# CANGA/ELMKernels

Hardware: AMD Instinct MI355X
Metric: gridcell-timesteps/sec (higher is better)
Workload: dtype f64

## Files before the change

### elmkernels_amd/csrc/elmk_albedo_col.h

```cpp
#pragma once
#include "elmk_dev.h"

namespace elmk {

#ifndef LV
#define LV(f, lev) S->f[(int64_t)(lev) * ld + c]
#endif

constexpr double SN_MIN_SNW = 1.0e-30;
constexpr double SA_MPE = 1.e-06;
constexpr double SA_EXTKN = 0.30;

__device__ __forceinline__ int alb_main_column(const DevState* __restrict__ S, const int64_t c, const int64_t ld, const Land& L)
{
  const double coszen = S->coszen[c];
  const double elai = S->elai[c];

  S->nrad[c] = 1;
  S->tlai_z[c] = elai;

  if (!(coszen > 0.0)) return -1;

  const double h2osno = S->h2osno[c];
  const int snl = S->snl[c];

  double albsod[2], albsoi[2];
  {
    const double albice[2] = {0.8, 0.55};
    const double alblak[2] = {0.60, 0.40};
    const double alblakwi[2] = {0.10, 0.10};
    if (L.ltype == istsoil || L.ltype == istcrop) {
      const int col = S->isoicol[c];
      const double inc = dmax(0.11 - 0.40 * LV(h2osoi_vol, 0), 0.0);
#pragma unroll
      for (int ib = 0; ib < 2; ib++) {
        albsod[ib] = dmin(S->albsat[col][ib] + inc, S->albdry[col][ib]);
        albsoi[ib] = albsod[ib];
      }
    } else if (L.ltype == istice || L.ltype == istice_mec) {
#pragma unroll
      for (int ib = 0; ib < 2; ib++) {
        albsod[ib] = albice[ib];
        albsoi[ib] = albsod[ib];
      }
    } else if (L.ltype == istdlak && snl == 0) {
      const double t_grnd = S->t_grnd[c];
      const double sicefr = 1.0 - elmk_exp(-95.6 * (TFRZ - t_grnd) / TFRZ);
#pragma unroll
      for (int ib = 0; ib < 2; ib++) {
        albsod[ib] = sicefr * alblak[ib] + (1.0 - sicefr) * dmax(alblakwi[ib], 0.05 / (dmax(0.001, coszen) + 0.15));
        albsoi[ib] = sicefr * alblak[ib] + (1.0 - sicefr) * dmax(alblakwi[ib], 0.10);
      }
    } else {
#pragma unroll
      for (int ib = 0; ib < 2; ib++) {
        albsod[ib] = alblak[ib];
        albsoi[ib] = albsod[ib];
      }
    }
  }


  LV(albsod, 0) = albsod[0];
  LV(albsod, 1) = albsod[1];
  LV(albsoi, 0) = albsoi[0];
  LV(albsoi, 1) = albsoi[1];
  if (h2osno > SN_MIN_SNW) return snl == 0 ? 1 : snl;
  return 0;
}

}
```

### elmkernels_amd/csrc/elmk_albedo_fin.h

```cpp
#pragma once
#include "elmk_dev.h"
#include "elmk_albedo_col.h"

namespace elmk {

struct AlbFwd {
  double albsod[2], albsoi[2], albsnd[2], albsni[2], albgrd[2], albgri[2];
  double albd[2], albi[2], ftdd[2], ftid[2], ftii[2], fabd[2], fabi[2];
  double fsun_z, fabd_sun_z, fabd_sha_z, fabi_sun_z, fabi_sha_z;
};

__device__ __forceinline__ void alb_ground(const DevState* __restrict__ S, const int64_t c, const int64_t ld, const bool day,
                                           const double frac_sno, const double (&albsod)[2], const double (&albsoi)[2],
                                           const double (&sd_alb)[2], const double (&si_alb)[2], AlbFwd& a)
{
#pragma unroll
  for (int ib = 0; ib < 2; ib++) {
    double o_sod = 0.0, o_soi = 0.0, o_snd = 0.0, o_sni = 0.0, g_d = 0.0, g_i = 0.0;
    if (day) {
      g_d = albsod[ib] * (1.0 - frac_sno) + sd_alb[ib] * frac_sno;
      g_i = albsoi[ib] * (1.0 - frac_sno) + si_alb[ib] * frac_sno;
      o_sod = albsod[ib];
      o_soi = albsoi[ib];
      o_snd = sd_alb[ib];
// ... 172 lines not shown
        fabi_sha_z = fabi_sha[ib] / ((1.0 - fsun_z) * laisum);
        const double extkb = twostext;
        vcmaxcintsun = (1.0 - elmk_exp(-(SA_EXTKN + extkb) * elai)) / (SA_EXTKN + extkb);
        vcmaxcintsha = (1.0 - elmk_exp(-SA_EXTKN * elai)) / SA_EXTKN - vcmaxcintsun;
        if (elai > 0.0) {
          vcmaxcintsun = vcmaxcintsun / (fsun_z * elai);
          vcmaxcintsha = vcmaxcintsha / ((1.0 - fsun_z) * elai);
        } else {
          vcmaxcintsun = 0.0;
          vcmaxcintsha = 0.0;
        }
      }
    }
  } else {
#pragma unroll
    for (int ib = 0; ib < 2; ++ib) {
      fabd[ib] = 0.0;
      fabi[ib] = 0.0;
      fabi_sun[ib] = 0.0;
      fabi_sha[ib] = 0.0;
      ftdd[ib] = 1.0;
      ftid[ib] = 0.0;
      ftii[ib] = 1.0;
      albd[ib] = albgrd[ib];
      albi[ib] = albgri[ib];
    }
  }
#pragma unroll
  for (int ib = 0; ib < 2; ib++) {
    LV(albd, ib) = albd[ib];
    LV(albi, ib) = albi[ib];
    LV(ftdd, ib) = ftdd[ib];
    LV(ftid, ib) = ftid[ib];
    LV(ftii, ib) = ftii[ib];
    LV(fabd, ib) = fabd[ib];
    LV(fabi, ib) = fabi[ib];
    LV(fabi_sun, ib) = fabi_sun[ib];
    LV(fabi_sha, ib) = fabi_sha[ib];
  }
  S->vcmaxcintsun[c] = vcmaxcintsun;
  S->vcmaxcintsha[c] = vcmaxcintsha;
  S->fsun_z[c] = fsun_z;
  S->fabd_sun_z[c] = fabd_sun_z;
  S->fabd_sha_z[c] = fabd_sha_z;
  S->fabi_sun_z[c] = fabi_sun_z;
  S->fabi_sha_z[c] = fabi_sha_z;
}

struct AlbIn {
  bool day, snicar;
  double coszen, elai, esai, frac_sno, vcmaxcintsun, vcmaxcintsha;
  double albsod[2], albsoi[2], sd_alb[2], si_alb[2];
};
__device__ __forceinline__ AlbIn alb_final_inputs(const DevState* __restrict__ S, const int64_t c, const int64_t ld, const double frac_sno_in,
                                                  const double h2osno_in)
{
  AlbIn x;
  x.coszen = S->coszen[c];
  x.elai = S->elai[c];
  x.vcmaxcintsun = 0.0;
  x.vcmaxcintsha = (1.0 - elmk_exp(-SA_EXTKN * x.elai)) / SA_EXTKN;
  if (x.elai > 0.0) {
    x.vcmaxcintsha /= x.elai;
  } else {
    x.vcmaxcintsha = 0.0;
  }
  x.day = x.coszen > 0.0;
  x.snicar = false;
  x.esai = 0.0;
  x.frac_sno = 0.0;
  x.albsod[0] = x.albsod[1] = x.albsoi[0] = x.albsoi[1] = 0.0;
  x.sd_alb[0] = x.sd_alb[1] = x.si_alb[0] = x.si_alb[1] = 0.0;
  if (x.day) {
    x.esai = S->esai[c];
    x.frac_sno = frac_sno_in;
    x.albsod[0] = LV(albsod, 0);
    x.albsod[1] = LV(albsod, 1);
    x.albsoi[0] = LV(albsoi, 0);
    x.albsoi[1] = LV(albsoi, 1);
    if (h2osno_in > SN_MIN_SNW) {
      const gptr<const double> o = S->alb_snow + c;
      x.snicar = true;
      x.sd_alb[0] = __builtin_nontemporal_load(o);
      x.sd_alb[1] = __builtin_nontemporal_load(o + ld);
      x.si_alb[0] = __builtin_nontemporal_load(o + (int64_t)14 * ld);
      x.si_alb[1] = __builtin_nontemporal_load(o + (int64_t)15 * ld);
    } else if (h2osno_in < SN_MIN_SNW && h2osno_in > 0.0) {
      x.sd_alb[0] = x.si_alb[0] = x.albsoi[0];
      x.sd_alb[1] = x.si_alb[1] = x.albsoi[1];
    }
  }
  return x;
}
__device__ __forceinline__ void alb_flux_abs_all(const DevState* __restrict__ S, const int64_t c, const int64_t ld, const Land& L,
                                                 const AlbIn& x, double (&flx)[6][4])
{
  const gptr<const double> o = S->alb_snow + c;
#pragma unroll
  for (int i = 0; i < 6; i++) {
    double sdf[2] = {0.0, 0.0}, sif[2] = {0.0, 0.0};
    if (x.snicar) {
      sdf[0] = __builtin_nontemporal_load(o + (int64_t)(2 + 2 * i) * ld);
      sdf[1] = __builtin_nontemporal_load(o + (int64_t)(3 + 2 * i) * ld);
      sif[0] = __builtin_nontemporal_load(o + (int64_t)(16 + 2 * i) * ld);
      sif[1] = __builtin_nontemporal_load(o + (int64_t)(17 + 2 * i) * ld);
    }
    alb_flux_abs_level(L, x.day, x.frac_sno, x.albsod, x.albsoi, x.sd_alb, x.si_alb, sdf, sif, flx[i][0], flx[i][1], flx[i][2], flx[i][3]);
    LV(flx_absdv, i) = flx[i][0];
    LV(flx_absdn, i) = flx[i][1];
    LV(flx_absiv, i) = flx[i][2];
    LV(flx_absin, i) = flx[i][3];
  }
}

}
```

### elmkernels_amd/csrc/elmk_api.cpp

```cpp
#include "elmk.h"

#include <hip/hip_runtime.h>

#include <cmath>
#include <cstddef>
#include <cstdio>
#include <cstdlib>
#include <algorithm>
#include <cstring>
#include <dlfcn.h>
#include <string>
#include <vector>

#include "elmk_dev.h"
#include "elmk_kernels.h"
#include "elmk_maps.h"

using namespace elmk;

namespace {

struct FieldDesc {
  const char* name;
  int dtype;
// ... 476 lines not shown
  }
  if (side.fork) (void)hipEventDestroy(side.fork);
  for (hipEvent_t e : done)
    if (e) (void)hipEventDestroy(e);
  if (upload) (void)hipStreamDestroy(upload);
  if (own) (void)hipStreamDestroy(own);
  return ELMK_OK;
}

const char* elmk_last_error(const elmk_ctx* ctx) { return ctx ? ctx->err.c_str() : g_create_error.c_str(); }

int elmk_set_stream(elmk_ctx* ctx, void* hip_stream)
{
  if (int rc = enter(ctx)) return rc;
  HIPCHK(hipStreamSynchronize(ctx->stream));
  ctx->stream = hip_stream ? (hipStream_t)hip_stream : ctx->own_stream;
  return ELMK_OK;
}

namespace {
int drop_graphs(elmk_ctx* ctx)
{
  HIPCHK(hipStreamSynchronize(ctx->stream));
  for (GraphSlot& g : ctx->graph) g.drop();
  return ELMK_OK;
}

int set_col_dayl(elmk_ctx* ctx, bool on)
{
  if (ctx->side.col_dayl == on) return ELMK_OK;
  if (int rc = drop_graphs(ctx)) return rc;
  ctx->side.col_dayl = on;
  return ELMK_OK;
}

int refuse_capture(elmk_ctx* ctx, const char* msg)
{
  hipStreamCaptureStatus cap = hipStreamCaptureStatusNone;
  if (hip_fail(ctx, hipStreamIsCapturing(ctx->stream, &cap), "hipStreamIsCapturing")) return ELMK_E_HIP;
  return cap != hipStreamCaptureStatusNone ? invalid(ctx, msg) : ELMK_OK;
}
}

int elmk_set_graph(elmk_ctx* ctx, int on)
{
  if (int rc = enter(ctx)) return rc;
  ctx->use_graph = on != 0;
  return ctx->use_graph ? ELMK_OK : drop_graphs(ctx);
}

int elmk_set_option(elmk_ctx* ctx, int option, int value)
{
  if (int rc = enter(ctx)) return rc;
  if (option != ELMK_OPT_CF_HALF_WORKGROUPS) return invalid(ctx, "elmk_set_option: unknown option");
  int cus = 0;
  HIPCHK(hipDeviceGetAttribute(&cus, hipDeviceAttributeMultiprocessorCount, ctx->dev));
  const int want = value ? (cus > 0 ? cus : 256) : 0;
  if (want != ctx->side.cf_half_groups) {
    if (int rc = drop_graphs(ctx)) return rc;
    ctx->side.cf_half_groups = want;
  }
  return ELMK_OK;
}

int elmk_sync(elmk_ctx* ctx)
{
  if (int rc = enter(ctx)) return rc;
  HIPCHK(hipStreamSynchronize(ctx->stream));
  return ELMK_OK;
}

int64_t elmk_ncols(const elmk_ctx* ctx) { return ctx ? ctx->ncols : -1; }
int64_t elmk_level_stride(const elmk_ctx* ctx) { return ctx ? ctx->ld : -1; }
int64_t elmk_device_bytes(const elmk_ctx* ctx)
{
  if (!ctx) return -1;
  size_t n = ctx->arena.bytes() + ctx->staging.bytes() + ctx->scratch.bytes() + ctx->snicar.bytes() + ctx->snowage.bytes() + ctx->d.bytes() +
             ctx->run.mem.bytes() + ctx->grid.mem.bytes() + ctx->ogrid.mem.bytes() + ctx->sw.czf.bytes() + ctx->run.rec.bytes() +
             ctx->ds.topo.bytes() + ctx->ds.gmem.bytes() + ctx->accum_table.bytes() + ctx->aer.mem.bytes();
  for (const elmk_ctx::HistEntry& e : ctx->hist) n += e.cells ? e.acc.bytes() : 0;
  for (const elmk_ctx::AccumEntry& e : ctx->accum) n += e.val.bytes();
  return (int64_t)n;
}

int elmk_num_fields(void) { return ELMK_NUM_FIELDS; }
const char* elmk_field_name(int field) { return field_ok(field) ? g_fields[field].name : nullptr; }
int elmk_field_id(const char* name)
{
  if (!name) return -1;
  for (int f = 0; f < ELMK_NUM_FIELDS; f++)
    if (strcmp(name, g_fields[f].name) == 0) return f;
  return -1;
}
int elmk_field_info(int field, int* nlev, int* dtype)
{
  if (!field_ok(field)) return ELMK_E_INVALID;
  if (nlev) *nlev = g_fields[field].nlev;
  if (dtype) *dtype = g_fields[field].dtype;
  return ELMK_OK;
}

static int xfer_rows(elmk_ctx* ctx, char* dev, int64_t ld, int es, int nlev, void* host, int64_t col0, int64_t n, int layout, bool up)
{
  if (layout == ELMK_LAYOUT_SOA || nlev == 1) {
    if (up)
      HIPCHK(hipMemcpy2DAsync(dev + (size_t)col0 * es, (size_t)ld * es, host, (size_t)n * es, (size_t)n * es, nlev, hipMemcpyHostToDevice,
// ... 2207 lines not shown
```

### elmkernels_amd/csrc/elmk_kernels.h

```cpp
#pragma once

#include <hip/hip_runtime.h>
#include <stdint.h>

#include "elmk.h"
#include "elmk_solar.h"

namespace elmk {

struct DevState;

constexpr int ELMK_NSIDE = 5;
struct SideStreams {
  hipStream_t s[ELMK_NSIDE];
  hipEvent_t fork;
  hipEvent_t join[ELMK_NSIDE];
  int cf_half_groups;
  bool one_stream;
  bool col_dayl;
};

void launch_frac_wet(const DevState* S, int64_t n, hipStream_t st);
void launch_albedo_snicar(const DevState* S, int64_t n, hipStream_t st, const SideStreams* side, bool fused = false);
unsigned launch_albedo_snicar_part(const DevState* S, int64_t n, hipStream_t st);
void launch_canopy_hydrology(const DevState* S, int64_t n, double dt, hipStream_t st);
void launch_surface_radiation(const DevState* S, int64_t n, hipStream_t st);
void launch_canopy_temperature(const DevState* S, int64_t n, hipStream_t st);
constexpr int GIVEN_FUSED = 1 << 8;
void launch_bareground_fluxes(const DevState* S, int64_t n, hipStream_t st, int given = 0);
void launch_canopy_fluxes(const DevState* S, int64_t n, double dt, hipStream_t st, int given = 0, const SideStreams* side = nullptr);
constexpr int ELMK_FUSED_NSTAGE = 5;
void launch_fused_stage(const DevState* S, int64_t n, double dt, hipStream_t st, const SideStreams* side, int stage);
void launch_bareground_list(const DevState* S, int64_t n, hipStream_t st);
void launch_soil_temperature(const DevState* S, int64_t n, double dt, hipStream_t st);
void launch_snow_hydrology(const DevState* S, int64_t n, double dt, hipStream_t st);
constexpr int ELMK_CONS_NPART = 512;
void launch_surface_fluxes(const DevState* S, int64_t n, double dt, hipStream_t st);
void launch_init_timestep(const DevState* S, int64_t n, hipStream_t st);
void launch_initialize_state(const DevState* S, int64_t n, hipStream_t st);
struct DsParams {
  const double* hc;
  const double* hf;
  double* lg;
  double lapse, lapse_lw, lw_limit;
};
void launch_get_forcing(const DevState* S, int64_t n, const double* wt1, const double* wt2, int qbot_is_rh, hipStream_t st,
                        const double* czf = nullptr, const DsParams* ds = nullptr);
void launch_phenology(const DevState* S, int64_t n, double wt1, double wt2, hipStream_t st);
void launch_conservation(const DevState* S, int64_t n, int64_t ld, double dt, const double* diag, double* part, double* out,
                         hipStream_t st);

void launch_cols_to_soa(const void* staging, void* field, int elem, int nlev, int64_t ld, int64_t col0, int64_t n,
                        hipStream_t st);
void launch_soa_to_cols(const void* field, void* staging, int elem, int nlev, int64_t ld, int64_t col0, int64_t n,
                        hipStream_t st);
constexpr int ELMK_F32_STORED = 16;
void launch_fill(void* field, int dtype, int nlev, int64_t ld, int64_t ncols, double value, hipStream_t st);
void launch_tile(void* field, int dtype, int nlev, int64_t ld, int64_t ncols, int64_t nbase, uint64_t seed,
                 int field_id, int mode, double amp, hipStream_t st);
void launch_flag_reduce(const uint32_t* flags, int64_t n, uint32_t* or_out, long long* first_bad, hipStream_t st);
void launch_copy(const double* src, double* dst, int64_t n, hipStream_t st, int shape = 0);
constexpr int COPY_JOBS_MAX = 16;
struct CopyJobs {
  const double* src[COPY_JOBS_MAX];
  double* dst[COPY_JOBS_MAX];
  int64_t end[COPY_JOBS_MAX];
  int n;
};
void launch_copy_multi(const CopyJobs& J, hipStream_t st);
void launch_math_eval(int fn, const double* x, const double* y, double* out, int64_t n, hipStream_t st);
// ... 107 lines not shown
```

### elmkernels_amd/csrc/elmk_snicar.h

```cpp
#pragma once
#include "elmk_dev.h"
#include "elmk_albedo_col.h"

namespace elmk {

constexpr int SN_RDS_MAX_TBL = 1500, SN_RDS_MIN_TBL = 30;
constexpr double SN_EXP_MIN = 4.5399929762484854e-05;

struct SnowOut {
  double alb[2];
  double fabs_[6][2];
};

template <int NL>
__device__ __forceinline__ void snicar_band(const DevState* __restrict__ S, const int64_t c, const int64_t ld, const int pass,
                                            const int bnd, const double mu_not, const int snl, const double h2osno,
                                            const double albsoi_b, double& albedo, double (&fl)[6], uint32_t& err)
{
  constexpr int snl_top = 5 - NL;
  const gptr<const double> tab = S->snicar;
  const double difgauspt[8] = {0.9894009, 0.9445750, 0.8656312, 0.7554044, 0.6178762, 0.4580168, 0.2816036, 0.0950125};
  const double difgauswt[8] = {0.0271525, 0.0622535, 0.0951585, 0.1246290, 0.1495960, 0.1691565, 0.1826034, 0.1894506};
  const double puny = 1.0e-11;
  const double c0 = 0.0, c1 = 1.0, c3 = 3.0, c4 = 4.0, cp5 = 0.5, cp75 = 0.75, c1p5 = 1.5, trmin = 0.001;
// ... 226 lines not shown

template <int NL, class FA, class FF>
__device__ __forceinline__ void snicar_combine_from(const int pass, const double mu_not, const int rds_top, const FA band_albedo,
                                                    const FF band_flux, SnowOut& out)
{
  constexpr int snl_top = 5 - NL;
  const double w1 = (pass == 0) ? 0.49352158521175 : 0.58581507618433;
  const double w2 = (pass == 0) ? 0.18099494230665 : 0.20156903770812;
  const double w3 = (pass == 0) ? 0.12094898498813 : 0.10917889346386;
  const double w4 = (pass == 0) ? 0.20453448749347 : 0.10343699264369;
  const double flx_wgt[5] = {1.0, w1, w2, w3, w4};
  double alb_nir_sum = 0.0, wgt_sum = 0.0;
  double nir_sum[6] = {0.0, 0.0, 0.0, 0.0, 0.0, 0.0};
  out.alb[0] = band_albedo(0);
#pragma unroll
  for (int i = 0; i < 6; i++) {
    out.fabs_[i][0] = band_flux(0, i);
    out.fabs_[i][1] = 0.0;
  }
#pragma unroll
  for (int b = 1; b < 5; b++) {
    alb_nir_sum += flx_wgt[b] * band_albedo(b);
    wgt_sum += flx_wgt[b];
#pragma unroll
    for (int i = 0; i < 6; i++) {
      const double f = band_flux(b, i);
      if (i >= snl_top) nir_sum[i] += flx_wgt[b] * f;
    }
  }
  out.alb[1] = alb_nir_sum / wgt_sum;
#pragma unroll
  for (int i = 0; i < 6; i++) {
    if (i >= snl_top) out.fabs_[i][1] = nir_sum[i] / wgt_sum;
  }
  if (pass == 0 && mu_not < 0.2588) {
    const double sza_c1 = 0.085730 + (-0.630883) * mu_not + 1.303723 * elmk_sq(mu_not);
    const double sza_c0 = 1.467291 + (-3.338043) * mu_not + 6.807489 * elmk_sq(mu_not);
    const double sza_factor = sza_c1 * (elmk_log10(rds_top * 1.0) - 6.0) + sza_c0;
    const double flx_sza_adjust = out.alb[1] * (sza_factor - 1.0) * wgt_sum;
    out.alb[1] *= sza_factor;
    out.fabs_[snl_top][1] -= flx_sza_adjust;
  }
}

template <int NL>
__device__ __forceinline__ void snicar_combine(const int g0, const int pass, const double mu_not, const int rds_top,
                                               const double albedo, const double (&fl)[6], SnowOut& out)
{
  snicar_combine_from<NL>(
      pass, mu_not, rds_top, [&](const int b) { return __shfl(albedo, g0 + b, 64); },
      [&](const int b, const int i) { return __shfl(fl[i], g0 + b, 64); }, out);
}

template <int NL>
__device__ __forceinline__ void snicar_workgroup(const DevState* __restrict__ S, const uint32_t block, const uint32_t nblocks)
{
  uint32_t count = ELMK_LIST_COUNT(S, LIST_ALB_0 + NL);
  if ((int64_t)count > S->ld) count = (uint32_t)S->ld;
  if ((uint64_t)block * (blockDim.x >> 6) * 6u >= count) return;
  elmk_math_lds_init<false>();
  const int64_t ld = S->ld;
  const gptr<const int32_t> list = S->lists + (int64_t)(LIST_ALB_0 + NL) * ld;
  constexpr int snl_top = NLEVSNO - NL;
  const int lane = threadIdx.x & 63;
  const int slot = lane / 10, task = lane - slot * 10;
  const int pass = task / 5, bnd = task - pass * 5;
  const int g0 = lane - bnd;
  const uint32_t nwaves = nblocks * (blockDim.x >> 6);
  for (uint32_t w = block * (blockDim.x >> 6) + (threadIdx.x >> 6); (uint64_t)w * 6u < count; w += nwaves) {
    const uint32_t q = w * 6u + (uint32_t)slot;
    const bool valid = slot < 6 && q < count;
    const int64_t c = list[valid ? q : w * 6u];
    uint32_t err = 0;
    const double mu_not = dmax(S->coszen[c], 0.01);
    const int snl = S->snl[c];
    const double h2osno = S->h2osno[c];
    const double albsoi_b = LV(albsoi, bnd == 0 ? 0 : 1);
    double albedo, fl[6];
    snicar_band<NL>(S, c, ld, pass, bnd, mu_not, snl, h2osno, albsoi_b, albedo, fl, err);
    int rds_top = (snl == 0) ? (int)round(SNW_RDS_MIN) : (int)round(LV(snw_rds, snl_top));
    rds_top = rds_top < SN_RDS_MIN_TBL ? SN_RDS_MIN_TBL : (rds_top > SN_RDS_MAX_TBL ? SN_RDS_MAX_TBL : rds_top);
    SnowOut out;
    snicar_combine<NL>(g0, pass, mu_not, rds_top, albedo, fl, out);
    if (valid && bnd == 0) {
      const gptr<double> o = S->alb_snow + (int64_t)(pass * 14) * ld + c;
      o[0] = out.alb[0];
      o[ld] = out.alb[1];
#pragma unroll
      for (int i = 0; i < 6; i++) {
        o[(int64_t)(2 + 2 * i) * ld] = out.fabs_[i][0];
        o[(int64_t)(3 + 2 * i) * ld] = out.fabs_[i][1];
      }
    }
    if (valid && err) atomicOr(ELMK_GENERIC(&S->err_flags[c]), err);
  }
}


}
```

### elmkernels_amd/csrc/k_albedo_snicar.hip

```cpp
#define ELMK_MATH_LDS 1
#include "elmk_dev.h"
#include "elmk_kernels.h"
#include "elmk_albedo_col.h"
#include "elmk_snicar.h"
#include "elmk_albedo_fin.h"

namespace elmk {



constexpr int ALB_CLASSIFY_THREADS = 1024;
__global__ __launch_bounds__(ALB_CLASSIFY_THREADS) void k_alb_classify(const DevState* __restrict__ S)
{
  const Land L = S->land;
  if (L.ltype == istdlak) elmk_math_lds_init<false>();
  const int64_t c = (int64_t)blockIdx.x * blockDim.x + threadIdx.x;
  const int64_t ld = S->ld;
  if (L.urbpoi) return;
  const bool inside = c < S->ncols;
  int nl = -1;
  if (inside) nl = alb_main_column(S, c, ld, L);
  block_classify_append<5>(S->lists, ld, S->counters, LIST_ALB_1, nl >= 1 ? nl - 1 : -1, (int32_t)c);
}

template <int NL>
__global__ __launch_bounds__(256, 2) void k_alb_snicar(const DevState* __restrict__ S)
{
  snicar_workgroup<NL>(S, blockIdx.x, gridDim.x);
}
template <int NL>
static void launch_snicar_deep(const DevState* S, const unsigned capped, const int64_t n, hipStream_t st)
{
  hipLaunchKernelGGL(k_alb_snicar<NL>, dim3(capped), dim3(256), 0, st, S);
}
constexpr int ALB_DEEP_PER_QUEUE = 1024;
__global__ __launch_bounds__(256, 2) void k_alb_snicar_deep(const DevState* __restrict__ S, const unsigned per_queue)
{
  const unsigned q = blockIdx.x / per_queue, b = blockIdx.x - q * per_queue;
  switch (q) {
    case 0: snicar_workgroup<5>(S, b, per_queue); break;
    case 1: snicar_workgroup<4>(S, b, per_queue); break;
    case 2: snicar_workgroup<3>(S, b, per_queue); break;
    default: snicar_workgroup<2>(S, b, per_queue);
  }
}
static void launch_snicar_deep_all(const DevState* S, const unsigned capped, hipStream_t st)
{
  const unsigned per_queue = capped < (unsigned)ALB_DEEP_PER_QUEUE ? capped : (unsigned)ALB_DEEP_PER_QUEUE;
  hipLaunchKernelGGL(k_alb_snicar_deep, dim3(4u * per_queue), dim3(256), 0, st, S, per_queue);
}

__global__ __launch_bounds__(256) void k_alb_final(const DevState* __restrict__ S)
{
  elmk_math_lds_init<false>();
  const int64_t c = (int64_t)blockIdx.x * blockDim.x + threadIdx.x;
  const int64_t ld = S->ld;
  const Land L = S->land;
  if (blockIdx.x == 0 && threadIdx.x < 6) {
    ELMK_LIST_COUNT(S, LIST_ALB_0 + threadIdx.x) = 0u;
    ELMK_LIST_HEAD(S, LIST_ALB_0 + threadIdx.x) = 0u;
  }
  if (L.urbpoi || c >= S->ncols) return;
  const AlbIn x = alb_final_inputs(S, c, ld, S->frac_sno[c], S->h2osno[c]);
  AlbFwd a;
  double flx[6][4];
  alb_ground(S, c, ld, x.day, x.frac_sno, x.albsod, x.albsoi, x.sd_alb, x.si_alb, a);
  alb_flux_abs_all(S, c, ld, L, x, flx);
  alb_two_stream(S, c, ld, L, x.day, x.coszen, x.elai, x.esai, x.vcmaxcintsun, x.vcmaxcintsha, a);
}

void launch_albedo_snicar(const DevState* S, int64_t n, hipStream_t st, const SideStreams* side, bool fused)
{
  if (n <= 0) return;
  const dim3 block(256);
  const unsigned full = (unsigned)((n + 255) / 256);
  const unsigned want = (unsigned)((n + 23) / 24);
  const unsigned capped = want < 4096u ? want : 4096u;
  if (!fused)
    hipLaunchKernelGGL(k_alb_classify, dim3((unsigned)((n + ALB_CLASSIFY_THREADS - 1) / ALB_CLASSIFY_THREADS)), dim3(ALB_CLASSIFY_THREADS), 0, st, S);
  if (n < 262144) {
    if (side->one_stream) {
      launch_snicar_deep<5>(S, capped, n, st);
      launch_snicar_deep<4>(S, capped, n, st);
      launch_snicar_deep<3>(S, capped, n, st);
      launch_snicar_deep<2>(S, capped, n, st);
      hipLaunchKernelGGL(k_alb_snicar<1>, dim3(capped), block, 0, st, S);
    } else {
      (void)hipEventRecord(side->fork, st);
      for (int i = 0; i < 4; i++) (void)hipStreamWaitEvent(side->s[i], side->fork, 0);
      launch_snicar_deep<5>(S, capped, n, st);
      launch_snicar_deep<4>(S, capped, n, side->s[0]);
      launch_snicar_deep<3>(S, capped, n, side->s[1]);
      launch_snicar_deep<2>(S, capped, n, side->s[2]);
      hipLaunchKernelGGL(k_alb_snicar<1>, dim3(capped), block, 0, side->s[3], S);
      for (int i = 0; i < 4; i++) {
        (void)hipEventRecord(side->join[i], side->s[i]);
        (void)hipStreamWaitEvent(st, side->join[i], 0);
      }
    }
  } else {
    launch_snicar_deep_all(S, capped, st);
    hipLaunchKernelGGL(k_alb_snicar<1>, dim3(capped), block, 0, st, S);
  }
  if (!fused) hipLaunchKernelGGL(k_alb_final, dim3(full), block, 0, st, S);
}

unsigned launch_albedo_snicar_part(const DevState* S, int64_t n, hipStream_t st)
{
  if (n <= 0) return 0u;
  const unsigned want = (unsigned)((n + 23) / 24);
  const unsigned capped = want < 4096u ? want : 4096u;
  launch_snicar_deep_all(S, capped, st);
  return capped;
}

}
```

### elmkernels_amd/state.py

```python
import ctypes as C

import numpy as np

from . import _lib as L
from .downscale import DS_MODES, LAPSE, LAPSE_LW, LW_LIMIT
from .shortwave import SW_COSZEN, SW_MODES, SW_REFERENCE

DTYPES = {0: np.float64, 1: np.int32, 2: np.uint8, 3: np.uint32}
LAYOUT_COL_MAJOR, LAYOUT_SOA = 0, 1
OPT_CF_HALF_WORKGROUPS = 1
HIST_AVG, HIST_SUM, HIST_MAX, HIST_MIN, HIST_INST = range(5)
HIST_OPS = {"avg": HIST_AVG, "sum": HIST_SUM, "max": HIST_MAX, "min": HIST_MIN, "inst": HIST_INST}
HIST_MAX_TAPES, HIST_MAX_ENTRIES = 4, 64
CLASS_PROGNOSTIC, CLASS_SURFACE, CLASS_FORCING, CLASS_DIAGNOSTIC = range(4)
CLASS_NAMES = ("prognostic", "surface", "forcing", "diagnostic")
RUN_QBOT_IS_RH, RUN_HISTORY, RUN_ACCUM, RUN_AEROSOL = 1, 2, 4, 8
ACCUM_RUNMEAN, ACCUM_TIMEAVG, ACCUM_RUNACCUM = range(3)
ACCUM_KINDS = {"runmean": ACCUM_RUNMEAN, "timeavg": ACCUM_TIMEAVG, "runaccum": ACCUM_RUNACCUM}
ACCUM_MAX_ENTRIES = 16
RUN_STEP_DTYPE = np.dtype([("decday", np.float64), ("doy", np.int32), ("forc_slot", np.int32), ("forc_wt1", np.float64, (8,)),
                           ("forc_wt2", np.float64, (8,)), ("month1", np.int32), ("month2", np.int32), ("month_wt1", np.float64),
                           ("month_wt2", np.float64)], align=True)
SERIES_FORCING = ("atm_tbot", "atm_pbot", "atm_qbot", "atm_flds", "atm_fsds", "atm_prec", "atm_wind")
SERIES_PHENOLOGY = ("mlai", "msai", "mhtop", "mhbot")

PSN_FIELDS = (
    "fnr act25 kcha koha cpha vcmaxha jmaxha tpuha lmrha vcmaxhd jmaxhd tpuhd lmrhd lmrse qe theta_cj "
    "bbbopt mbbopt c3psn slatop leafcn flnr fnitr dleaf smpso smpsc tc_stress"
).split()
ALB_SOURCES = ["rholvis", "rholnir", "rhosvis", "rhosnir", "taulvis", "taulnir", "tausvis", "tausnir", "xl"]


def _p(a):
    return a.ctypes.data_as(C.c_void_p)


def _csr_args(ptr, col, w, rows_name):
    ptr = np.ascontiguousarray(ptr, dtype=np.int64).reshape(-1)
    col = np.ascontiguousarray(col, dtype=np.int32).reshape(-1)
    w = np.ascontiguousarray(w, dtype=np.float64).reshape(-1)
    if ptr.size < 2 or col.size != w.size or ptr[-1] != col.size:
        raise ValueError(f"ptr must be [{rows_name} + 1] with ptr[-1] == len(col) == len(w)")
    return ptr.size - 1, ptr, col, w


def field_table():
    lib = L.load()
    out = {}
    for i in range(lib.elmk_num_fields()):
        nlev, dt = C.c_int(), C.c_int()
        lib.elmk_field_info(i, C.byref(nlev), C.byref(dt))
        out[lib.elmk_field_name(i).decode()] = (i, nlev.value, DTYPES[dt.value])
    return out


def field_class(name, lib_path=None):
    lib = L.load(lib_path)
    fid = lib.elmk_field_id(name.encode()) if isinstance(name, str) else int(name)
    c = lib.elmk_field_class(fid)
    if c < 0:
        raise KeyError(name)
    return c

# ... 714 lines not shown
```

### include/elmk.h

```cpp
#ifndef ELMK_H
#define ELMK_H

#include <stdint.h>

#ifdef __cplusplus
extern "C" {
#endif

typedef struct elmk_ctx elmk_ctx;

enum {
  ELMK_NLEVSNO = 5,
  ELMK_NLEVGRND = 15,
  ELMK_NLEVTOT = 20,
  ELMK_NUMRAD = 2,
  ELMK_NLEVCAN = 1,
  ELMK_NUMRAD_SNW = 5,
  ELMK_SNO_NBR_AER = 8,
  ELMK_MXPFT = 25,
  ELMK_NSOILCOL = 20,
  ELMK_MIE_N = 1471,
  ELMK_PSN_NPARAM = 27,
  ELMK_ALB_NPARAM = 9
};
// ... 17 lines not shown
#define ELMK_FIELD(name, T, nlev) ELMK_FIELD_##name,
#include "elmk_fields.def"
#undef ELMK_FIELD
  ELMK_FIELD_err_flags,
  ELMK_NUM_FIELDS
} elmk_field;

enum {
  ELMK_ERR_SURFRAD_LAYER_SUM = 1u << 0,
  ELMK_ERR_CANFLX_FORC_HGT = 1u << 1,
  ELMK_ERR_PSN_NEG_GS = 1u << 2,
  ELMK_ERR_PSN_QUADRATIC = 1u << 3,
  ELMK_ERR_PSN_BRENT_BRACKET = 1u << 4,
  ELMK_ERR_ALB_CANOPY_LAYERS = 1u << 5,
  ELMK_ERR_SNICAR_RDS = 1u << 6,
  ELMK_ERR_SNICAR_FLAG = 1u << 7,
  ELMK_ERR_SNICAR_NEG_ABS = 1u << 8,
  ELMK_ERR_SNICAR_ENERGY = 1u << 9,
  ELMK_ERR_SNICAR_ALBEDO = 1u << 10,
  ELMK_WARN_PSN_BALL_BERRY = 1u << 11,
  ELMK_WARN_SNOW_WATER_OOB = 1u << 12,
  ELMK_WARN_SNOW_COMBINE_OOB = 1u << 13,
  ELMK_ERR_SNOW_DIVIDE_RDS = 1u << 14,
  ELMK_ERR_SNOW_AGE_DRFRESH = 1u << 15
};
#define ELMK_ERR_FATAL_MASK 0xC7FFu

typedef struct {
  const double *ss_alb_oc1, *asm_prm_oc1, *ext_cff_mss_oc1;
  const double *ss_alb_oc2, *asm_prm_oc2, *ext_cff_mss_oc2;
  const double *ss_alb_dst1, *asm_prm_dst1, *ext_cff_mss_dst1;
  const double *ss_alb_dst2, *asm_prm_dst2, *ext_cff_mss_dst2;
  const double *ss_alb_dst3, *asm_prm_dst3, *ext_cff_mss_dst3;
  const double *ss_alb_dst4, *asm_prm_dst4, *ext_cff_mss_dst4;
  const double *ss_alb_snw_drc, *asm_prm_snw_drc, *ext_cff_mss_snw_drc;
  const double *ss_alb_snw_dfs, *asm_prm_snw_dfs, *ext_cff_mss_snw_dfs;
  const double *ss_alb_bc1, *asm_prm_bc1, *ext_cff_mss_bc1;
  const double *ss_alb_bc2, *asm_prm_bc2, *ext_cff_mss_bc2;
  const double *bcenh;
} elmk_snicar_tables;

typedef struct {
  int32_t field;
  int32_t mode;
  double amp;
} elmk_perturb;

int elmk_create(int64_t ncols, int device_id, elmk_ctx **out);
int elmk_destroy(elmk_ctx *ctx);
const char *elmk_last_error(const elmk_ctx *ctx);
int elmk_set_stream(elmk_ctx *ctx, void *hip_stream);
int elmk_sync(elmk_ctx *ctx);
int elmk_set_graph(elmk_ctx *ctx, int on);
enum { ELMK_OPT_CF_HALF_WORKGROUPS = 1 };
int elmk_set_option(elmk_ctx *ctx, int option, int value);
int64_t elmk_ncols(const elmk_ctx *ctx);
int64_t elmk_level_stride(const elmk_ctx *ctx);
int64_t elmk_device_bytes(const elmk_ctx *ctx);

int elmk_num_fields(void);
const char *elmk_field_name(int field);
int elmk_field_id(const char *name);
int elmk_field_info(int field, int *nlev, int *dtype);
int elmk_state_real_bytes(void);

int elmk_upload(elmk_ctx *ctx, int field, const void *host, int64_t col0, int64_t n, int layout);
int elmk_download(elmk_ctx *ctx, int field, void *host, int64_t col0, int64_t n, int layout);
int elmk_fill(elmk_ctx *ctx, int field, double value);
void *elmk_device_ptr(elmk_ctx *ctx, int field);
int elmk_tile_columns(elmk_ctx *ctx, int64_t nbase, uint64_t seed, int nrules, const elmk_perturb *rules);
int elmk_snapshot_fields(elmk_ctx *ctx, const int *fields, int nfields);
int elmk_restore_fields(elmk_ctx *ctx);

int elmk_set_land(elmk_ctx *ctx, int ltype, int ctype, int vtype, int urbpoi, int lakpoi);
int elmk_set_scalars(elmk_ctx *ctx, double dewmx, int oldfflag, double dayl, double max_dayl);
int elmk_set_pft(elmk_ctx *ctx, const double *psn, const double *alb, const double *z0mr, const double *displar);
int elmk_set_soilcolor(elmk_ctx *ctx, const double *albsat , const double *albdry );
int elmk_set_snicar(elmk_ctx *ctx, const elmk_snicar_tables *t);
int elmk_set_snow_age_tables(elmk_ctx *ctx, const double *tau, const double *kappa, const double *drdt0);

int elmk_set_column_geography(elmk_ctx *ctx, const double *lat_r, const double *lon_r);
int elmk_solar_geometry(elmk_ctx *ctx, double dt_seconds, double decday, int doy);
int elmk_download_day_length(elmk_ctx *ctx, double *dayl, double *max_dayl);
int elmk_clear_column_geography(elmk_ctx *ctx);

enum { ELMK_HIST_AVG = 0, ELMK_HIST_SUM = 1, ELMK_HIST_MAX = 2, ELMK_HIST_MIN = 3, ELMK_HIST_INST = 4 };
#define ELMK_HIST_MAX_TAPES 4
#define ELMK_HIST_MAX_ENTRIES 64
int elmk_history_add(elmk_ctx *ctx, int tape, int field, int op);
int elmk_history_accumulate(elmk_ctx *ctx);
int elmk_history_reset(elmk_ctx *ctx, int tape);
int elmk_history_count(elmk_ctx *ctx, int tape, int64_t *nsamples);
int elmk_history_read(elmk_ctx *ctx, int entry, double *host, int64_t col0, int64_t n, int layout);
int elmk_history_clear(elmk_ctx *ctx);

typedef struct {
  double decday;
  int32_t doy;
  int32_t forc_slot;
  double forc_wt1[8], forc_wt2[8];
  int32_t month1, month2;
  double month_wt1, month_wt2;
} elmk_run_step;
enum { ELMK_RUN_QBOT_IS_RH = 1, ELMK_RUN_HISTORY = 2 };
#define ELMK_RUN_ACCUM 4
#define ELMK_RUN_AEROSOL 8
int elmk_run_reserve(elmk_ctx *ctx, int forcing_slots, int max_steps);
// ... 135 lines not shown
```

Baseline: 464.4 million.

## Fuse single-layer SNICAR columns into tiled albedo finalize kernel via LDS staging

Single-snow-layer columns are no longer queued for a separate SNICAR kernel. A new tiled kernel compacts those columns per 256-thread block, runs the SNICAR solve in-block, keeps the needed albedo and top-layer absorption rows in shared memory, and then does the albedo finalization in the same kernel. This removes one launch and the global round trip through alb_snow for the common one-layer case. The cost is a large LDS footprint that may limit occupancy, and load imbalance inside each tile. The old staged path stays available behind a new option.

```diff
diff --git a/elmkernels_amd/csrc/elmk_albedo_col.h b/elmkernels_amd/csrc/elmk_albedo_col.h
--- a/elmkernels_amd/csrc/elmk_albedo_col.h
+++ b/elmkernels_amd/csrc/elmk_albedo_col.h
@@ -11,6 +11,13 @@
 constexpr double SA_MPE = 1.e-06;
 constexpr double SA_EXTKN = 0.30;
 
+__device__ __forceinline__ bool alb_sunlit(const double coszen) { return coszen > 0.0; }
+__device__ __forceinline__ int alb_snicar_layers(const double h2osno, const int snl)
+{
+  if (h2osno > SN_MIN_SNW) return snl == 0 ? 1 : snl;
+  return 0;
+}
+
 __device__ __forceinline__ int alb_main_column(const DevState* __restrict__ S, const int64_t c, const int64_t ld, const Land& L)
 {
   const double coszen = S->coszen[c];
@@ -19,7 +26,7 @@
   S->nrad[c] = 1;
   S->tlai_z[c] = elai;
 
-  if (!(coszen > 0.0)) return -1;
+  if (!alb_sunlit(coszen)) return -1;
 
   const double h2osno = S->h2osno[c];
   const int snl = S->snl[c];
@@ -65,8 +72,7 @@
   LV(albsod, 1) = albsod[1];
   LV(albsoi, 0) = albsoi[0];
   LV(albsoi, 1) = albsoi[1];
-  if (h2osno > SN_MIN_SNW) return snl == 0 ? 1 : snl;
-  return 0;
+  return alb_snicar_layers(h2osno, snl);
 }
 
 }
diff --git a/elmkernels_amd/csrc/elmk_albedo_fin.h b/elmkernels_amd/csrc/elmk_albedo_fin.h
--- a/elmkernels_amd/csrc/elmk_albedo_fin.h
+++ b/elmkernels_amd/csrc/elmk_albedo_fin.h
@@ -248,8 +248,9 @@
   double coszen, elai, esai, frac_sno, vcmaxcintsun, vcmaxcintsha;
   double albsod[2], albsoi[2], sd_alb[2], si_alb[2];
 };
+template <class FS>
 __device__ __forceinline__ AlbIn alb_final_inputs(const DevState* __restrict__ S, const int64_t c, const int64_t ld, const double frac_sno_in,
-                                                  const double h2osno_in)
+                                                  const double h2osno_in, const FS snow)
 {
   AlbIn x;
   x.coszen = S->coszen[c];
@@ -261,7 +262,7 @@
   } else {
     x.vcmaxcintsha = 0.0;
   }
-  x.day = x.coszen > 0.0;
+  x.day = alb_sunlit(x.coszen);
   x.snicar = false;
   x.esai = 0.0;
   x.frac_sno = 0.0;
@@ -275,12 +276,11 @@
     x.albsoi[0] = LV(albsoi, 0);
     x.albsoi[1] = LV(albsoi, 1);
     if (h2osno_in > SN_MIN_SNW) {
-      const gptr<const double> o = S->alb_snow + c;
       x.snicar = true;
-      x.sd_alb[0] = __builtin_nontemporal_load(o);
-      x.sd_alb[1] = __builtin_nontemporal_load(o + ld);
-      x.si_alb[0] = __builtin_nontemporal_load(o + (int64_t)14 * ld);
-      x.si_alb[1] = __builtin_nontemporal_load(o + (int64_t)15 * ld);
+      x.sd_alb[0] = snow(0);
+      x.sd_alb[1] = snow(1);
+      x.si_alb[0] = snow(14);
+      x.si_alb[1] = snow(15);
     } else if (h2osno_in < SN_MIN_SNW && h2osno_in > 0.0) {
       x.sd_alb[0] = x.si_alb[0] = x.albsoi[0];
       x.sd_alb[1] = x.si_alb[1] = x.albsoi[1];
@@ -288,18 +288,18 @@
   }
   return x;
 }
+template <class FS>
 __device__ __forceinline__ void alb_flux_abs_all(const DevState* __restrict__ S, const int64_t c, const int64_t ld, const Land& L,
-                                                 const AlbIn& x, double (&flx)[6][4])
-{
-  const gptr<const double> o = S->alb_snow + c;
+                                                 const AlbIn& x, double (&flx)[6][4], const FS snow)
+{
 #pragma unroll
   for (int i = 0; i < 6; i++) {
     double sdf[2] = {0.0, 0.0}, sif[2] = {0.0, 0.0};
     if (x.snicar) {
-      sdf[0] = __builtin_nontemporal_load(o + (int64_t)(2 + 2 * i) * ld);
-      sdf[1] = __builtin_nontemporal_load(o + (int64_t)(3 + 2 * i) * ld);
-      sif[0] = __builtin_nontemporal_load(o + (int64_t)(16 + 2 * i) * ld);
-      sif[1] = __builtin_nontemporal_load(o + (int64_t)(17 + 2 * i) * ld);
+      sdf[0] = snow(2 + 2 * i);
+      sdf[1] = snow(3 + 2 * i);
+      sif[0] = snow(16 + 2 * i);
+      sif[1] = snow(17 + 2 * i);
     }
     alb_flux_abs_level(L, x.day, x.frac_sno, x.albsod, x.albsoi, x.sd_alb, x.si_alb, sdf, sif, flx[i][0], flx[i][1], flx[i][2], flx[i][3]);
     LV(flx_absdv, i) = flx[i][0];
@@ -309,4 +309,21 @@
   }
 }
 
-}
+struct alb_snow_reader {
+  gptr<const double> o;
+  int64_t ld;
+  __device__ __forceinline__ alb_snow_reader(const DevState* __restrict__ S, const int64_t c, const int64_t ld_) : o(S->alb_snow + c), ld(ld_) {}
+  __device__ __forceinline__ double operator()(const int k) const { return __builtin_nontemporal_load(o + (int64_t)k * ld); }
+};
+__device__ __forceinline__ AlbIn alb_final_inputs(const DevState* __restrict__ S, const int64_t c, const int64_t ld, const double frac_sno_in,
+                                                  const double h2osno_in)
+{
+  return alb_final_inputs(S, c, ld, frac_sno_in, h2osno_in, alb_snow_reader(S, c, ld));
+}
+__device__ __forceinline__ void alb_flux_abs_all(const DevState* __restrict__ S, const int64_t c, const int64_t ld, const Land& L,
+                                                 const AlbIn& x, double (&flx)[6][4])
+{
+  alb_flux_abs_all(S, c, ld, L, x, flx, alb_snow_reader(S, c, ld));
+}
+
+}
diff --git a/elmkernels_amd/csrc/elmk_api.cpp b/elmkernels_amd/csrc/elmk_api.cpp
--- a/elmkernels_amd/csrc/elmk_api.cpp
+++ b/elmkernels_amd/csrc/elmk_api.cpp
@@ -552,6 +552,14 @@
 int elmk_set_option(elmk_ctx* ctx, int option, int value)
 {
   if (int rc = enter(ctx)) return rc;
+  if (option == ELMK_OPT_ALB_STAGED) {
+    const bool want = value != 0;
+    if (want != ctx->side.alb_staged) {
+      if (int rc = drop_graphs(ctx)) return rc;
+      ctx->side.alb_staged = want;
+    }
+    return ELMK_OK;
+  }
   if (option != ELMK_OPT_CF_HALF_WORKGROUPS) return invalid(ctx, "elmk_set_option: unknown option");
   int cus = 0;
   HIPCHK(hipDeviceGetAttribute(&cus, hipDeviceAttributeMultiprocessorCount, ctx->dev));
diff --git a/elmkernels_amd/csrc/elmk_kernels.h b/elmkernels_amd/csrc/elmk_kernels.h
--- a/elmkernels_amd/csrc/elmk_kernels.h
+++ b/elmkernels_amd/csrc/elmk_kernels.h
@@ -16,6 +16,7 @@
   hipEvent_t fork;
   hipEvent_t join[ELMK_NSIDE];
   int cf_half_groups;
+  bool alb_staged;
   bool one_stream;
   bool col_dayl;
 };
diff --git a/elmkernels_amd/csrc/elmk_snicar.h b/elmkernels_amd/csrc/elmk_snicar.h
--- a/elmkernels_amd/csrc/elmk_snicar.h
+++ b/elmkernels_amd/csrc/elmk_snicar.h
@@ -302,25 +302,20 @@
       [&](const int b, const int i) { return __shfl(fl[i], g0 + b, 64); }, out);
 }
 
-template <int NL>
-__device__ __forceinline__ void snicar_workgroup(const DevState* __restrict__ S, const uint32_t block, const uint32_t nblocks)
-{
-  uint32_t count = ELMK_LIST_COUNT(S, LIST_ALB_0 + NL);
-  if ((int64_t)count > S->ld) count = (uint32_t)S->ld;
-  if ((uint64_t)block * (blockDim.x >> 6) * 6u >= count) return;
-  elmk_math_lds_init<false>();
+template <int NL, class FC, class FO>
+__device__ __forceinline__ void snicar_queue(const DevState* __restrict__ S, const uint32_t count, const uint32_t wave0,
+                                             const uint32_t nwaves, const FC column_at, const FO store)
+{
   const int64_t ld = S->ld;
-  const gptr<const int32_t> list = S->lists + (int64_t)(LIST_ALB_0 + NL) * ld;
   constexpr int snl_top = NLEVSNO - NL;
   const int lane = threadIdx.x & 63;
   const int slot = lane / 10, task = lane - slot * 10;
   const int pass = task / 5, bnd = task - pass * 5;
   const int g0 = lane - bnd;
-  const uint32_t nwaves = nblocks * (blockDim.x >> 6);
-  for (uint32_t w = block * (blockDim.x >> 6) + (threadIdx.x >> 6); (uint64_t)w * 6u < count; w += nwaves) {
+  for (uint32_t w = wave0; (uint64_t)w * 6u < count; w += nwaves) {
     const uint32_t q = w * 6u + (uint32_t)slot;
     const bool valid = slot < 6 && q < count;
-    const int64_t c = list[valid ? q : w * 6u];
+    const int64_t c = column_at(valid ? q : w * 6u);
     uint32_t err = 0;
     const double mu_not = dmax(S->coszen[c], 0.01);
     const int snl = S->snl[c];
@@ -332,19 +327,33 @@
     rds_top = rds_top < SN_RDS_MIN_TBL ? SN_RDS_MIN_TBL : (rds_top > SN_RDS_MAX_TBL ? SN_RDS_MAX_TBL : rds_top);
     SnowOut out;
     snicar_combine<NL>(g0, pass, mu_not, rds_top, albedo, fl, out);
-    if (valid && bnd == 0) {
-      const gptr<double> o = S->alb_snow + (int64_t)(pass * 14) * ld + c;
-      o[0] = out.alb[0];
-      o[ld] = out.alb[1];
-#pragma unroll
-      for (int i = 0; i < 6; i++) {
-        o[(int64_t)(2 + 2 * i) * ld] = out.fabs_[i][0];
-        o[(int64_t)(3 + 2 * i) * ld] = out.fabs_[i][1];
-      }
-    }
+    if (valid && bnd == 0) store(c, pass, out);
     if (valid && err) atomicOr(ELMK_GENERIC(&S->err_flags[c]), err);
   }
 }
 
-
-}
+template <int NL>
+__device__ __forceinline__ void snicar_workgroup(const DevState* __restrict__ S, const uint32_t block, const uint32_t nblocks)
+{
+  uint32_t count = ELMK_LIST_COUNT(S, LIST_ALB_0 + NL);
+  if ((int64_t)count > S->ld) count = (uint32_t)S->ld;
+  if ((uint64_t)block * (blockDim.x >> 6) * 6u >= count) return;
+  elmk_math_lds_init<false>();
+  const int64_t ld = S->ld;
+  const gptr<const int32_t> list = S->lists + (int64_t)(LIST_ALB_0 + NL) * ld;
+  snicar_queue<NL>(
+      S, count, block * (blockDim.x >> 6) + (threadIdx.x >> 6), nblocks * (blockDim.x >> 6), [&](const uint32_t q) { return (int64_t)list[q]; },
+      [&](const int64_t c, const int pass, const SnowOut& out) {
+        const gptr<double> o = S->alb_snow + (int64_t)(pass * 14) * ld + c;
+        o[0] = out.alb[0];
+        o[ld] = out.alb[1];
+#pragma unroll
+        for (int i = 0; i < 6; i++) {
+          o[(int64_t)(2 + 2 * i) * ld] = out.fabs_[i][0];
+          o[(int64_t)(3 + 2 * i) * ld] = out.fabs_[i][1];
+        }
+      });
+}
+
+
+}
diff --git a/elmkernels_amd/csrc/k_albedo_snicar.hip b/elmkernels_amd/csrc/k_albedo_snicar.hip
--- a/elmkernels_amd/csrc/k_albedo_snicar.hip
+++ b/elmkernels_amd/csrc/k_albedo_snicar.hip
@@ -10,7 +10,7 @@
 
 
 constexpr int ALB_CLASSIFY_THREADS = 1024;
-__global__ __launch_bounds__(ALB_CLASSIFY_THREADS) void k_alb_classify(const DevState* __restrict__ S)
+__global__ __launch_bounds__(ALB_CLASSIFY_THREADS) void k_alb_classify(const DevState* __restrict__ S, const int queue_one)
 {
   const Land L = S->land;
   if (L.ltype == istdlak) elmk_math_lds_init<false>();
@@ -20,6 +20,7 @@
   const bool inside = c < S->ncols;
   int nl = -1;
   if (inside) nl = alb_main_column(S, c, ld, L);
+  if (nl == 1 && !queue_one) nl = 0;
   block_classify_append<5>(S->lists, ld, S->counters, LIST_ALB_1, nl >= 1 ? nl - 1 : -1, (int32_t)c);
 }
 
@@ -69,6 +70,76 @@
   alb_two_stream(S, c, ld, L, x.day, x.coszen, x.elai, x.esai, x.vcmaxcintsun, x.vcmaxcintsha, a);
 }
 
+constexpr int ALB_TILE = 256;
+constexpr int ALB_TILE_KEPT = 12;
+__host__ __device__ constexpr int alb_tile_row(const int k)
+{
+  const int pass = k / 14, r = k - pass * 14;
+  return r < 2 ? pass * 6 + r : (r >= 10 ? pass * 6 + r - 8 : -1);
+}
+__global__ __launch_bounds__(ALB_TILE, 4) void k_alb_tile(const DevState* __restrict__ S)
+{
+  __shared__ double s_snow[ALB_TILE_KEPT][ALB_TILE];
+  __shared__ uint16_t s_list[ALB_TILE];
+  __shared__ uint32_t s_wcnt[ALB_TILE / 64];
+  const int64_t ld = S->ld;
+  const Land L = S->land;
+  if (blockIdx.x == 0 && threadIdx.x < 6) {
+    ELMK_LIST_COUNT(S, LIST_ALB_0 + threadIdx.x) = 0u;
+    ELMK_LIST_HEAD(S, LIST_ALB_0 + threadIdx.x) = 0u;
+  }
+  if (L.urbpoi) return;
+  const int64_t c0 = (int64_t)blockIdx.x * ALB_TILE, c = c0 + threadIdx.x;
+  const bool inside = c < S->ncols;
+  const int lane = threadIdx.x & 63, wave = threadIdx.x >> 6;
+
+  double h2osno = 0.0;
+  bool one = false;
+  if (inside) {
+    h2osno = S->h2osno[c];
+    one = alb_sunlit(S->coszen[c]) && alb_snicar_layers(h2osno, S->snl[c]) == 1;
+  }
+  const unsigned long long m = __ballot(one);
+  if (lane == 0) s_wcnt[wave] = (uint32_t)__popcll(m);
+  elmk_math_lds_init<false>();
+  uint32_t base = 0u, count = 0u;
+#pragma unroll
+  for (int w = 0; w < ALB_TILE / 64; w++) {
+    const uint32_t n = s_wcnt[w];
+    base += w < wave ? n : 0u;
+    count += n;
+  }
+  if (one) s_list[base + (uint32_t)__popcll(m & ((1ull << lane) - 1ull))] = (uint16_t)threadIdx.x;
+  __syncthreads();
+
+  snicar_queue<1>(
+      S, count, (uint32_t)wave, ALB_TILE / 64, [&](const uint32_t q) { return c0 + (int64_t)s_list[q]; },
+      [&](const int64_t cq, const int pass, const SnowOut& out) {
+        const int t = (int)(cq - c0);
+        s_snow[pass * 6 + 0][t] = out.alb[0];
+        s_snow[pass * 6 + 1][t] = out.alb[1];
+        s_snow[pass * 6 + 2][t] = out.fabs_[4][0];
+        s_snow[pass * 6 + 3][t] = out.fabs_[4][1];
+        s_snow[pass * 6 + 4][t] = out.fabs_[5][0];
+        s_snow[pass * 6 + 5][t] = out.fabs_[5][1];
+      });
+  __syncthreads();
+
+  if (!inside) return;
+  const alb_snow_reader deep(S, c, ld);
+  const auto snow = [&](const int k) -> double {
+    if (!one) return deep(k);
+    const int r = alb_tile_row(k);
+    return r < 0 ? 0.0 : s_snow[r < 0 ? 0 : r][threadIdx.x];
+  };
+  const AlbIn x = alb_final_inputs(S, c, ld, S->frac_sno[c], h2osno, snow);
+  AlbFwd a;
+  double flx[6][4];
+  alb_ground(S, c, ld, x.day, x.frac_sno, x.albsod, x.albsoi, x.sd_alb, x.si_alb, a);
+  alb_flux_abs_all(S, c, ld, L, x, flx, snow);
+  alb_two_stream(S, c, ld, L, x.day, x.coszen, x.elai, x.esai, x.vcmaxcintsun, x.vcmaxcintsha, a);
+}
+
 void launch_albedo_snicar(const DevState* S, int64_t n, hipStream_t st, const SideStreams* side, bool fused)
 {
   if (n <= 0) return;
@@ -76,15 +147,17 @@
   const unsigned full = (unsigned)((n + 255) / 256);
   const unsigned want = (unsigned)((n + 23) / 24);
   const unsigned capped = want < 4096u ? want : 4096u;
+  const bool queue_one = fused || side->alb_staged;
   if (!fused)
-    hipLaunchKernelGGL(k_alb_classify, dim3((unsigned)((n + ALB_CLASSIFY_THREADS - 1) / ALB_CLASSIFY_THREADS)), dim3(ALB_CLASSIFY_THREADS), 0, st, S);
+    hipLaunchKernelGGL(k_alb_classify, dim3((unsigned)((n + ALB_CLASSIFY_THREADS - 1) / ALB_CLASSIFY_THREADS)), dim3(ALB_CLASSIFY_THREADS), 0, st, S,
+                       (int)queue_one);
   if (n < 262144) {
     if (side->one_stream) {
       launch_snicar_deep<5>(S, capped, n, st);
       launch_snicar_deep<4>(S, capped, n, st);
       launch_snicar_deep<3>(S, capped, n, st);
       launch_snicar_deep<2>(S, capped, n, st);
-      hipLaunchKernelGGL(k_alb_snicar<1>, dim3(capped), block, 0, st, S);
+      if (queue_one) hipLaunchKernelGGL(k_alb_snicar<1>, dim3(capped), block, 0, st, S);
     } else {
       (void)hipEventRecord(side->fork, st);
       for (int i = 0; i < 4; i++) (void)hipStreamWaitEvent(side->s[i], side->fork, 0);
@@ -92,7 +165,7 @@
       launch_snicar_deep<4>(S, capped, n, side->s[0]);
       launch_snicar_deep<3>(S, capped, n, side->s[1]);
       launch_snicar_deep<2>(S, capped, n, side->s[2]);
-      hipLaunchKernelGGL(k_alb_snicar<1>, dim3(capped), block, 0, side->s[3], S);
+      if (queue_one) hipLaunchKernelGGL(k_alb_snicar<1>, dim3(capped), block, 0, side->s[3], S);
       for (int i = 0; i < 4; i++) {
         (void)hipEventRecord(side->join[i], side->s[i]);
         (void)hipStreamWaitEvent(st, side->join[i], 0);
@@ -100,9 +173,14 @@
     }
   } else {
     launch_snicar_deep_all(S, capped, st);
-    hipLaunchKernelGGL(k_alb_snicar<1>, dim3(capped), block, 0, st, S);
+    if (queue_one) hipLaunchKernelGGL(k_alb_snicar<1>, dim3(capped), block, 0, st, S);
   }
-  if (!fused) hipLaunchKernelGGL(k_alb_final, dim3(full), block, 0, st, S);
+  if (fused) return;
+  if (queue_one) {
+    hipLaunchKernelGGL(k_alb_final, dim3(full), block, 0, st, S);
+  } else {
+    hipLaunchKernelGGL(k_alb_tile, dim3(full), dim3(ALB_TILE), 0, st, S);
+  }
 }
 
 unsigned launch_albedo_snicar_part(const DevState* S, int64_t n, hipStream_t st)
diff --git a/elmkernels_amd/state.py b/elmkernels_amd/state.py
--- a/elmkernels_amd/state.py
+++ b/elmkernels_amd/state.py
@@ -9,6 +9,7 @@
 DTYPES = {0: np.float64, 1: np.int32, 2: np.uint8, 3: np.uint32}
 LAYOUT_COL_MAJOR, LAYOUT_SOA = 0, 1
 OPT_CF_HALF_WORKGROUPS = 1
+OPT_ALB_STAGED = 2
 HIST_AVG, HIST_SUM, HIST_MAX, HIST_MIN, HIST_INST = range(5)
 HIST_OPS = {"avg": HIST_AVG, "sum": HIST_SUM, "max": HIST_MAX, "min": HIST_MIN, "inst": HIST_INST}
 HIST_MAX_TAPES, HIST_MAX_ENTRIES = 4, 64
diff --git a/include/elmk.h b/include/elmk.h
--- a/include/elmk.h
+++ b/include/elmk.h
@@ -93,7 +93,7 @@
 int elmk_set_stream(elmk_ctx *ctx, void *hip_stream);
 int elmk_sync(elmk_ctx *ctx);
 int elmk_set_graph(elmk_ctx *ctx, int on);
-enum { ELMK_OPT_CF_HALF_WORKGROUPS = 1 };
+enum { ELMK_OPT_CF_HALF_WORKGROUPS = 1, ELMK_OPT_ALB_STAGED = 2 };
 int elmk_set_option(elmk_ctx *ctx, int option, int value);
 int64_t elmk_ncols(const elmk_ctx *ctx);
 int64_t elmk_level_stride(const elmk_ctx *ctx);
```

New measurement: 478.6 million (median of 6 runs). 3.1% higher.
